# sara-nl/2D-VQ-AE-2

Hardware: AMD Instinct MI355X
Metric: patches/sec (VQAE.forward: encoder -> VQ -> decoder) (higher is better)
Workload: dtype f32; 1 GPU; BASELINE configs[1] (cfg B): batch 256/GPU of 256x256x3 fp32 -> 32x32 codes, K=256, D=128, full forward; global_batch=256, parallelism=patch-sharded x1

## Files before the change

### 2d-vq-ae-2_amd/csrc/conv_wino.hip

```cpp
#include "kernels.h"
#include "mfma.h"

namespace {

using namespace vqae;

struct WinoK {
    const float* __restrict__ t1;
    const float* __restrict__ U;
    const float* __restrict__ w3;
    const float* __restrict__ w1n;
    float* xio;
    float* y2;
    int H, Wimg, M;
    float act_a, act_b, t_scale, t_b4, n_b1a, n_b1b, n_b2a, n_b2b;
};

constexpr int BPF = 6;

template <int C> struct WinoCfg {
    static constexpr int W = C >= 128 ? 32 : (C == 64 ? 64 : 128);
    static constexpr int NT = C == 256 ? 512 : 256;
    static constexpr int NW = NT / 64;
    static constexpr int PX = 4 * W;
    static constexpr int TILES = PX / 4;
    static constexpr int TC = W / 2;
    static constexpr int NS = C / 32;
    static constexpr int KS = C / 8;
    static constexpr int C4 = C / 4;
    static constexpr int RP = NT / C4;
    static constexpr int LDT = C + 4;
    static constexpr int NI = C >= 64 ? 2 : 1;
    static constexpr int WN = C / (32 * NI);
    static constexpr int MI = PX / ((NW / WN) * 32);
    static constexpr int LDS_BYTES = PX * LDT * 4;
    static constexpr int PREF = C <= 64 ? 1 : 0;
};

template <int C, int TAIL, int DT, bool WIDE>
__global__ __launch_bounds__((WinoCfg<C>::NT), 2)
void wino_trunk_kernel(const WinoK p) {
    using K = WinoCfg<C>;
    auto rnd = [](float v) -> float {
        if (DT == VQAE_DT_BF16) return (float)(__bf16)v;
        if (DT == VQAE_DT_F16) return (float)(_Float16)v;
        return v;
    };
    auto rnd4 = [&](f32x4 v) -> f32x4 {
        if (DT != VQAE_DT_F32) {
#pragma unroll
            for (int e = 0; e < 4; ++e) v[e] = rnd(v[e]);
        }
        return v;
    };
    constexpr int W = K::W, PX = K::PX, TC = K::TC, NS = K::NS, KS = K::KS, C4 = K::C4, RP = K::RP, LDT = K::LDT, WN = K::WN;
    constexpr int MI = K::MI, NI = K::NI;
    constexpr bool PREF = K::PREF && !WIDE;
    constexpr int STEPS = 4 * KS;
    extern __shared__ __attribute__((aligned(16))) float lds[];
    const int tid = threadIdx.x;
    const int lane = tid & 63;
    const int wave = __builtin_amdgcn_readfirstlane(tid >> 6);
    const int li = lane & 31, hh = lane >> 5;
    const int ns = wave % NS, mt = wave / NS;

    int tile_m;
    {
        const int nwg = gridDim.x, bid = blockIdx.x;
        const int q = nwg >> 3, r = nwg & 7, xcd = bid & 7;
        tile_m = (xcd < r ? xcd * (q + 1) : r * (q + 1) + (xcd - r) * q) + (bid >> 3);
    }
    const int Wimg = WIDE ? p.Wimg : W;
    const int cblocks = WIDE ? p.Wimg / W : 1;
    const int tpi = (p.H / 4) * cblocks;
    const int img = tile_m / tpi;
    const int rem = tile_m - img * tpi;
    const int row0 = 4 * (rem / cblocks);
    const int col0 = W * (rem % cblocks);
    const int hw = p.H * Wimg;
    const float* const xim = p.t1 + (int64_t)img * hw * C;

    const int cg = tid % C4;
    const int tj0 = tid / C4;
    int coff[2][4], roff[2][4];
#pragma unroll
    for (int s = 0; s < 2; ++s) {
#pragma unroll
        for (int j = 0; j < 4; ++j) {
            int c = col0 + 2 * (tj0 + RP * s) - 1 + j;
            c = WIDE ? (c < 0 ? c + Wimg : (c >= Wimg ? c - Wimg : c)) : (c & (W - 1));
            coff[s][j] = c * C + 4 * cg;
            int r = row0 + 2 * s - 1 + j;
            r = r < 0 ? r + p.H : (r >= p.H ? r - p.H : r);
            roff[s][j] = r * Wimg * C;
        }
    }

    const float* const ub = p.U + (int64_t)ns * (KS * 256) + 4 * lane;
    const float* const af = lds + (mt * 32 + li) * LDT + 4 * hh;

    f32x4 v[4][4], la[2][4], lb[2][4];
    auto tr_load = [&](int xi, int s_r) {
        const int ra = xi == 0 ? 0 : (xi == 2 ? 2 : 1);
        const int rb = xi == 0 ? 2 : (xi == 1 ? 2 : (xi == 2 ? 1 : 3));
#pragma unroll
        for (int s_c = 0; s_c < 2; ++s_c)
#pragma unroll
            for (int j = 0; j < 4; ++j) {
                la[s_c][j] = rnd4(*reinterpret_cast<const f32x4*>(xim + roff[s_r][ra] + coff[s_c][j]));
                lb[s_c][j] = rnd4(*reinterpret_cast<const f32x4*>(xim + roff[s_r][rb] + coff[s_c][j]));
            }
    };
    auto tr_combine = [&](int xi, int s_r) {
#pragma unroll
        for (int s_c = 0; s_c < 2; ++s_c)
#pragma unroll
            for (int j = 0; j < 4; ++j)
                v[2 * s_r + s_c][j] = xi == 1 ? la[s_c][j] + lb[s_c][j] : la[s_c][j] - lb[s_c][j];
    };
    tr_load(0, 0);
    tr_combine(0, 0);
    tr_load(0, 1);
    tr_combine(0, 1);

    const int wm = wave / WN, wn = wave % WN;
    const int64_t pix0 = ((int64_t)img * p.H + row0) * Wimg + col0 + tj0;
    float* xr[4];
    f32x4 res[16];
    f32x4 bt[2][4][NI];
    auto tail_prefetch = [&](const float* __restrict__ wsrc) {
        const float* b0 = wsrc + (wn * NI) * (KS * 256) + 4 * lane;
#pragma unroll
        for (int u = 0; u < 4; ++u)
#pragma unroll
            for (int ni = 0; ni < NI; ++ni) bt[0][u][ni] = *reinterpret_cast<const f32x4*>(b0 + ni * (KS * 256) + 256 * u);
    };

    f32x16 y00, y01, y10, y11;
#pragma unroll
    for (int r = 0; r < 16; ++r) { y00[r] = 0.f; y01[r] = 0.f; y10[r] = 0.f; y11[r] = 0.f; }
#pragma unroll
    for (int xi = 0; xi < 4; ++xi) {
        __builtin_amdgcn_sched_barrier(0);
        if (xi > 0) __syncthreads();
#pragma unroll
        for (int it = 0; it < 4; ++it) {
            const int tile = (it >> 1) * TC + tj0 + RP * (it & 1);
            float* dst = lds + tile * LDT + 4 * cg;
            *reinterpret_cast<f32x4*>(dst + 0 * K::TILES * LDT) = v[it][0] - v[it][2];
            *reinterpret_cast<f32x4*>(dst + 1 * K::TILES * LDT) = v[it][1] + v[it][2];
            *reinterpret_cast<f32x4*>(dst + 2 * K::TILES * LDT) = v[it][2] - v[it][1];
            *reinterpret_cast<f32x4*>(dst + 3 * K::TILES * LDT) = v[it][1] - v[it][3];
        }

        const float* const ux = ub + (int64_t)(4 * xi) * (C * C);
#define WB(s) (((s) / KS) * (C * C) + 256 * ((s) % KS))
        f32x4 bq[BPF];
#pragma unroll
        for (int s = 0; s < BPF; ++s)
            bq[s] = *reinterpret_cast<const f32x4*>(ux + WB(s));
        __syncthreads();
        if (PREF && xi < 3) tr_load(xi + 1, 0);
        f32x4 aq[2];
        aq[0] = *reinterpret_cast<const f32x4*>(af);
#pragma unroll
        for (int nu = 0; nu < 4; ++nu) {
            f32x16 acc;
#pragma unroll
            for (int r = 0; r < 16; ++r) acc[r] = 0.f;
#pragma unroll
            for (int u = 0; u < KS; ++u) {
                const int s = KS * nu + u;
                if (s + 1 < STEPS)
                    aq[(s + 1) & 1] = *reinterpret_cast<const f32x4*>(af + ((s + 1) / KS) * K::TILES * LDT + 8 * ((s + 1) % KS));
                const f32x4 b = bq[s % BPF];
                if (s + BPF < STEPS)
                    bq[s % BPF] = *reinterpret_cast<const f32x4*>(ux + WB(s + BPF));
                if (xi == 3 && s == STEPS - BPF) {
                    tail_prefetch(p.w3);
#pragma unroll
                    for (int r = 0; r < 4; ++r) xr[r] = p.xio + (pix0 + (int64_t)r * Wimg) * C + 4 * cg;
#pragma unroll
                    for (int i = 0; i < 16; ++i) res[i] = __builtin_nontemporal_load(reinterpret_cast<const f32x4*>(xr[(RP * i) / W] + ((RP * i) % W) * C));
                }
#pragma unroll
                for (int r = 0; r < 4; ++r)
                    acc = __builtin_amdgcn_mfma_f32_32x32x2f32(b[r], aq[s & 1][r], acc, 0, 0, 0);
                __builtin_amdgcn_sched_barrier(0);
            }
            const int ca0 = xi <= 2 ? 1 : 0, ca1 = xi == 0 ? 0 : (xi == 1 ? 1 : -1);
            const int cb0 = nu <= 2 ? 1 : 0, cb1 = nu == 0 ? 0 : (nu == 1 ? 1 : -1);
            if (ca0 * cb0 != 0) y00 = y00 + acc;
            if (ca0 * cb1 == 1) y01 = y01 + acc; else if (ca0 * cb1 == -1) y01 = y01 - acc;
            if (ca1 * cb0 == 1) y10 = y10 + acc; else if (ca1 * cb0 == -1) y10 = y10 - acc;
            if (ca1 * cb1 == 1) y11 = y11 + acc; else if (ca1 * cb1 == -1) y11 = y11 - acc;
            asm volatile("" : "+v"(y00), "+v"(y01), "+v"(y10), "+v"(y11));
        }
#undef WB
        if (xi < 3) {
            if (!PREF) tr_load(xi + 1, 0);
            tr_combine(xi + 1, 0); tr_load(xi + 1, 1); tr_combine(xi + 1, 1);
        }
    }

    __syncthreads();
    float* const T = lds;
    {
        const int tile = mt * 32 + li;
        const int px = (2 * (tile / TC)) * W + 2 * (tile % TC);
        float* const d = T + px * LDT + 32 * ns + 4 * hh;
#pragma unroll
        for (int g = 0; g < 4; ++g) {
            f32x4 o00, o01, o10, o11;
#pragma unroll
            for (int e = 0; e < 4; ++e) {
                o00[e] = rnd(elu_act(rnd(y00[4 * g + e]) + p.act_a) + p.act_b);
                o01[e] = rnd(elu_act(rnd(y01[4 * g + e]) + p.act_a) + p.act_b);
                o10[e] = rnd(elu_act(rnd(y10[4 * g + e]) + p.act_a) + p.act_b);
                o11[e] = rnd(elu_act(rnd(y11[4 * g + e]) + p.act_a) + p.act_b);
            }
            *reinterpret_cast<f32x4*>(d + 8 * g) = o00;
            *reinterpret_cast<f32x4*>(d + 8 * g + LDT) = o01;
            *reinterpret_cast<f32x4*>(d + 8 * g + W * LDT) = o10;
            *reinterpret_cast<f32x4*>(d + 8 * g + (W + 1) * LDT) = o11;
        }
    }
    __syncthreads();

    f32x16 acc[MI][NI];
    auto gemm_tail = [&](const float* __restrict__ wsrc) {
#pragma unroll
        for (int mi = 0; mi < MI; ++mi)
#pragma unroll
            for (int ni = 0; ni < NI; ++ni)
#pragma unroll
                for (int r = 0; r < 16; ++r) acc[mi][ni][r] = 0.f;
        const float* a0 = T + (wm * MI * 32 + li) * LDT + 4 * hh;
        const float* b0 = wsrc + (wn * NI) * (KS * 256) + 4 * lane;
        f32x4 a[2][MI];
#pragma unroll
        for (int mi = 0; mi < MI; ++mi) a[0][mi] = *reinterpret_cast<const f32x4*>(a0 + mi * 32 * LDT);
#pragma unroll
        for (int ug = 0; ug < KS / 4; ++ug) {
            if (ug + 1 < KS / 4) {
#pragma unroll
                for (int u = 0; u < 4; ++u)
#pragma unroll
                    for (int ni = 0; ni < NI; ++ni)
                        bt[(ug + 1) & 1][u][ni] = *reinterpret_cast<const f32x4*>(b0 + ni * (KS * 256) + 256 * (4 * (ug + 1) + u));
            }
#pragma unroll
            for (int u = 0; u < 4; ++u) {
                const int ks = 4 * ug + u;
                if (ks + 1 < KS) {
#pragma unroll
                    for (int mi = 0; mi < MI; ++mi)
                        a[(ks + 1) & 1][mi] = *reinterpret_cast<const f32x4*>(a0 + mi * 32 * LDT + 8 * (ks + 1));
                }
#pragma unroll
                for (int r = 0; r < 4; ++r)
#pragma unroll
                    for (int mi = 0; mi < MI; ++mi)
#pragma unroll
                        for (int ni = 0; ni < NI; ++ni)
                            acc[mi][ni] = __builtin_amdgcn_mfma_f32_32x32x2f32(bt[ug & 1][u][ni][r], a[ks & 1][mi][r], acc[mi][ni], 0, 0, 0);
            }
        }
    };
    auto acc_to_lds = [&]() {
#pragma unroll
        for (int ni = 0; ni < NI; ++ni)
#pragma unroll
            for (int mi = 0; mi < MI; ++mi)
#pragma unroll
                for (int g = 0; g < 4; ++g) {
                    f32x4 o;
#pragma unroll
                    for (int e = 0; e < 4; ++e) o[e] = acc[mi][ni][4 * g + e];
                    *reinterpret_cast<f32x4*>(T + (wm * MI * 32 + mi * 32 + li) * LDT + (wn * NI + ni) * 32 + 8 * g + 4 * hh) = o;
                }
    };
    float* const trow = T + tj0 * LDT + 4 * cg;

    gemm_tail(p.w3);
    if (TAIL == 2) tail_prefetch(p.w1n);
    __syncthreads();
    acc_to_lds();
    __syncthreads();
#pragma unroll
    for (int i = 0; i < 16; ++i) {
        f32x4 t = rnd4(*reinterpret_cast<const f32x4*>(trow + RP * i * LDT));
        t = t * p.t_scale;
        t = t + p.t_b4;
        t = t + res[i];
        __builtin_nontemporal_store(t, reinterpret_cast<f32x4*>(xr[(RP * i) / W] + ((RP * i) % W) * C));
        if (TAIL == 2) {
#pragma unroll
            for (int e = 0; e < 4; ++e) t[e] = rnd(elu_act(t[e] + p.n_b1a) + p.n_b1b);
            *reinterpret_cast<f32x4*>(trow + RP * i * LDT) = t;
        }
    }
    if constexpr (TAIL == 2) {
        __syncthreads();
        gemm_tail(p.w1n);
        __syncthreads();
        acc_to_lds();
        __syncthreads();
        float* yr[4];
#pragma unroll
        for (int r = 0; r < 4; ++r) yr[r] = p.y2 + (pix0 + (int64_t)r * Wimg) * C + 4 * cg;
#pragma unroll
        for (int i = 0; i < 16; ++i) {
            f32x4 t = *reinterpret_cast<const f32x4*>(trow + RP * i * LDT);
#pragma unroll
            for (int e = 0; e < 4; ++e) t[e] = elu_act(rnd(t[e]) + p.n_b2a) + p.n_b2b;
            __builtin_nontemporal_store(t, reinterpret_cast<f32x4*>(yr[(RP * i) / W] + ((RP * i) % W) * C));
        }
    }
}

template <int C>
__global__ __launch_bounds__((WinoCfg<C>::NT), 2)
void fixup_conv1_kernel(const float* __restrict__ x, const float* __restrict__ w1f, float pa, float pb, float aa, float ab,
                        float* __restrict__ y) {
    using K = WinoCfg<C>;
    constexpr int PX = K::PX, KS = K::KS, C4 = K::C4, RP = K::RP, LDT = K::LDT, WN = K::WN, MI = K::MI, NI = K::NI;
    extern __shared__ __attribute__((aligned(16))) float lds[];
    float* const T = lds;
    const int tid = threadIdx.x;
    const int lane = tid & 63;
    const int wave = __builtin_amdgcn_readfirstlane(tid >> 6);
    const int li = lane & 31, hh = lane >> 5;
    const int cg = tid % C4, p0 = tid / C4;
    const int64_t m0 = (int64_t)blockIdx.x * PX;
    const float* const xrow = x + (m0 + p0) * C + 4 * cg;
    float* const trow = T + p0 * LDT + 4 * cg;
    f32x4 v[16];
#pragma unroll
    for (int i = 0; i < 16; ++i) v[i] = *reinterpret_cast<const f32x4*>(xrow + (int64_t)(RP * i) * C);
#pragma unroll
    for (int i = 0; i < 16; ++i) {
#pragma unroll
        for (int e = 0; e < 4; ++e) v[i][e] = elu_act(v[i][e] + pa) + pb;
        *reinterpret_cast<f32x4*>(trow + RP * i * LDT) = v[i];
    }
    __syncthreads();
    const int wm = wave / WN, wn = wave % WN;
    f32x16 acc[MI][NI];
#pragma unroll
    for (int mi = 0; mi < MI; ++mi)
#pragma unroll
        for (int ni = 0; ni < NI; ++ni)
#pragma unroll
            for (int r = 0; r < 16; ++r) acc[mi][ni][r] = 0.f;
    {
        const float* a0 = T + (wm * MI * 32 + li) * LDT + 4 * hh;
        const float* b0 = w1f + (wn * NI) * (KS * 256) + 4 * lane;
        f32x4 a[2][MI], bq[2][NI];
#pragma unroll
        for (int mi = 0; mi < MI; ++mi) a[0][mi] = *reinterpret_cast<const f32x4*>(a0 + mi * 32 * LDT);
#pragma unroll
        for (int ni = 0; ni < NI; ++ni) bq[0][ni] = *reinterpret_cast<const f32x4*>(b0 + ni * (KS * 256));
#pragma unroll
        for (int u = 0; u < KS; ++u) {
            if (u + 1 < KS) {
#pragma unroll
                for (int mi = 0; mi < MI; ++mi) a[(u + 1) & 1][mi] = *reinterpret_cast<const f32x4*>(a0 + mi * 32 * LDT + 8 * (u + 1));
#pragma unroll
                for (int ni = 0; ni < NI; ++ni) bq[(u + 1) & 1][ni] = *reinterpret_cast<const f32x4*>(b0 + ni * (KS * 256) + 256 * (u + 1));
            }
#pragma unroll
            for (int r = 0; r < 4; ++r)
#pragma unroll
                for (int mi = 0; mi < MI; ++mi)
#pragma unroll
                    for (int ni = 0; ni < NI; ++ni)
                        acc[mi][ni] = __builtin_amdgcn_mfma_f32_32x32x2f32(bq[u & 1][ni][r], a[u & 1][mi][r], acc[mi][ni], 0, 0, 0);
        }
    }
    __syncthreads();
#pragma unroll
    for (int ni = 0; ni < NI; ++ni)
#pragma unroll
        for (int mi = 0; mi < MI; ++mi)
#pragma unroll
            for (int g = 0; g < 4; ++g) {
                f32x4 o;
#pragma unroll
                for (int e = 0; e < 4; ++e) o[e] = elu_act(acc[mi][ni][4 * g + e] + aa) + ab;
                *reinterpret_cast<f32x4*>(T + (wm * MI * 32 + mi * 32 + li) * LDT + (wn * NI + ni) * 32 + 8 * g + 4 * hh) = o;
            }
    __syncthreads();
    float* const yrow = y + (m0 + p0) * C + 4 * cg;
#pragma unroll
    for (int i = 0; i < 16; ++i)
        *reinterpret_cast<f32x4*>(yrow + (int64_t)(RP * i) * C) = *reinterpret_cast<const f32x4*>(trow + RP * i * LDT);
}

template <int C>
__global__ __launch_bounds__((WinoCfg<C>::NT), 2)
void fixup_conv1p_kernel(const float* __restrict__ x, const float* __restrict__ w1f, float pa, float pb, float aa, float ab,
                         float* __restrict__ y, const int n_tiles) {
    using K = WinoCfg<C>;
    constexpr int PX = K::PX, KS = K::KS, C4 = K::C4, RP = K::RP, LDT = K::LDT, WN = K::WN, MI = K::MI, NI = K::NI;
    extern __shared__ __attribute__((aligned(16))) float lds[];
    float* const T = lds;
    const int tid = threadIdx.x;
    const int lane = tid & 63;
    const int wave = __builtin_amdgcn_readfirstlane(tid >> 6);
    const int li = lane & 31, hh = lane >> 5;
    const int cg = tid % C4, p0 = tid / C4;
    const int wm = wave / WN, wn = wave % WN;
    float* const trow = T + p0 * LDT + 4 * cg;
    const float* const a0 = T + (wm * MI * 32 + li) * LDT + 4 * hh;
    const float* const b0 = w1f + (wn * NI) * (KS * 256) + 4 * lane;
    int tile = blockIdx.x;
    f32x4 v[16];
    if (tile < n_tiles) {
        const float* const xrow = x + ((int64_t)tile * PX + p0) * C + 4 * cg;
#pragma unroll
        for (int i = 0; i < 16; ++i) v[i] = __builtin_nontemporal_load(reinterpret_cast<const f32x4*>(xrow + (int64_t)(RP * i) * C));
    }
    for (; tile < n_tiles; tile += gridDim.x) {
#pragma unroll
        for (int i = 0; i < 16; ++i) {
#pragma unroll
            for (int e = 0; e < 4; ++e) v[i][e] = elu_act(v[i][e] + pa) + pb;
            *reinterpret_cast<f32x4*>(trow + RP * i * LDT) = v[i];
        }
        vqae::lds_barrier();
        const int nt = tile + gridDim.x;
        if (nt < n_tiles) {
            const float* const xrow = x + ((int64_t)nt * PX + p0) * C + 4 * cg;
#pragma unroll
            for (int i = 0; i < 16; ++i) v[i] = __builtin_nontemporal_load(reinterpret_cast<const f32x4*>(xrow + (int64_t)(RP * i) * C));
        }
        f32x16 acc[MI][NI];
#pragma unroll
        for (int mi = 0; mi < MI; ++mi)
#pragma unroll
            for (int ni = 0; ni < NI; ++ni)
#pragma unroll
                for (int r = 0; r < 16; ++r) acc[mi][ni][r] = 0.f;
        {
            f32x4 a[2][MI], bq[2][NI];
#pragma unroll
            for (int mi = 0; mi < MI; ++mi) a[0][mi] = *reinterpret_cast<const f32x4*>(a0 + mi * 32 * LDT);
#pragma unroll
            for (int ni = 0; ni < NI; ++ni) bq[0][ni] = *reinterpret_cast<const f32x4*>(b0 + ni * (KS * 256));
#pragma unroll 1
            for (int u2 = 0; u2 < KS; u2 += 2) {
#pragma unroll
                for (int uu = 0; uu < 2; ++uu) {
                    const int u = u2 + uu;
                    if (u + 1 < KS) {
#pragma unroll
                        for (int mi = 0; mi < MI; ++mi) a[(uu + 1) & 1][mi] = *reinterpret_cast<const f32x4*>(a0 + mi * 32 * LDT + 8 * (u + 1));
#pragma unroll
                        for (int ni = 0; ni < NI; ++ni) bq[(uu + 1) & 1][ni] = *reinterpret_cast<const f32x4*>(b0 + ni * (KS * 256) + 256 * (u + 1));
                    }
#pragma unroll
                    for (int r = 0; r < 4; ++r)
#pragma unroll
                        for (int mi = 0; mi < MI; ++mi)
#pragma unroll
                            for (int ni = 0; ni < NI; ++ni)
                                acc[mi][ni] = __builtin_amdgcn_mfma_f32_32x32x2f32(bq[uu & 1][ni][r], a[uu & 1][mi][r], acc[mi][ni], 0, 0, 0);
                }
            }
        }
        vqae::lds_barrier();
#pragma unroll
        for (int ni = 0; ni < NI; ++ni)
#pragma unroll
            for (int mi = 0; mi < MI; ++mi)
#pragma unroll
                for (int g = 0; g < 4; ++g) {
                    f32x4 o;
#pragma unroll
                    for (int e = 0; e < 4; ++e) o[e] = elu_act(acc[mi][ni][4 * g + e] + aa) + ab;
                    *reinterpret_cast<f32x4*>(T + (wm * MI * 32 + mi * 32 + li) * LDT + (wn * NI + ni) * 32 + 8 * g + 4 * hh) = o;
                }
        vqae::lds_barrier();
        float* const yrow = y + ((int64_t)tile * PX + p0) * C + 4 * cg;
#pragma unroll
        for (int i = 0; i < 16; ++i)
            *reinterpret_cast<f32x4*>(yrow + (int64_t)(RP * i) * C) = *reinterpret_cast<const f32x4*>(trow + RP * i * LDT);
        vqae::lds_barrier();
    }
}

__global__ void wino_weight_kernel(const float* __restrict__ w, int c, int dt, float* __restrict__ U) {
    const int i = blockIdx.x * blockDim.x + threadIdx.x;
    if (i >= c * c) return;
    float g[3][3], t[4][3];
#pragma unroll
    for (int a = 0; a < 3; ++a)
#pragma unroll
        for (int b = 0; b < 3; ++b) g[a][b] = vqae::round_dt(w[(int64_t)i * 9 + a * 3 + b], dt);
#pragma unroll
    for (int b = 0; b < 3; ++b) {
        t[0][b] = g[0][b];
        t[1][b] = 0.5f * (g[0][b] + g[1][b] + g[2][b]);
        t[2][b] = 0.5f * (g[0][b] - g[1][b] + g[2][b]);
        t[3][b] = g[2][b];
    }
    const int fo = frag_offset(i / c, i % c, c);
    const int64_t cc = (int64_t)c * c;
#pragma unroll
    for (int a = 0; a < 4; ++a) {
        U[(a * 4 + 0) * cc + fo] = t[a][0];
        U[(a * 4 + 1) * cc + fo] = 0.5f * (t[a][0] + t[a][1] + t[a][2]);
        U[(a * 4 + 2) * cc + fo] = 0.5f * (t[a][0] - t[a][1] + t[a][2]);
        U[(a * 4 + 3) * cc + fo] = t[a][2];
    }
}

__global__ void frag_weight_kernel(const float* __restrict__ w, int n_rows, int K, int sk, float* __restrict__ out) {
    const int i = blockIdx.x * blockDim.x + threadIdx.x;
    if (i >= n_rows * K) return;
    out[frag_offset(i / K, i % K, K, sk)] = w[i];
}

template <int C, int DT, bool WIDE>
int launch_wino_w(const WinoK& k, bool chain, hipStream_t stream) {
    using K = WinoCfg<C>;
    if (int rc = vqae::set_max_dynamic_lds((const void*)wino_trunk_kernel<C, 1, DT, WIDE>, K::LDS_BYTES)) return rc;
    if (int rc = vqae::set_max_dynamic_lds((const void*)wino_trunk_kernel<C, 2, DT, WIDE>, K::LDS_BYTES)) return rc;
    const unsigned grid = (unsigned)(k.M / K::PX);
    const double flops = 2.0 * (double)k.M * C * (4.0 * C + C + (chain ? C : 0));
    vqae::ProfScope prof(C >= 128 ? vqae::PROF_CONV3X3_TRUNK : vqae::PROF_NONE, stream, flops);
    if (chain) wino_trunk_kernel<C, 2, DT, WIDE><<<grid, K::NT, K::LDS_BYTES, stream>>>(k);
    else wino_trunk_kernel<C, 1, DT, WIDE><<<grid, K::NT, K::LDS_BYTES, stream>>>(k);
    prof.done();
    VQAE_LAUNCH_CHECK();
    return VQAE_OK;
}

template <int C, int DT = VQAE_DT_F32>
int launch_wino(const WinoK& k, bool chain, hipStream_t stream) {
    return k.Wimg == WinoCfg<C>::W ? launch_wino_w<C, DT, false>(k, chain, stream) : launch_wino_w<C, DT, true>(k, chain, stream);
}

}

namespace vqae {

bool wino_trunk_channels(int c, int dtype) { return dtype == VQAE_DT_F32 ? (c == 256 || c == 128 || c == 64 || c == 32) : c == 32; }

bool wino_trunk_supported(int c, int h, int w, int dtype) {
    if (!wino_trunk_channels(c, dtype)) return false;
    const int span = c >= 128 ? 32 : (c == 64 ? WinoCfg<64>::W : WinoCfg<32>::W);
    return w >= span && w % span == 0 && h >= 4 && h % 4 == 0;
}

size_t wino_weight_floats(int c) { return (size_t)16 * c * c; }

int wino_transform_weight(const float* w_oihw_dev, int c, int dtype, float* U_dev, hipStream_t stream) {
    wino_weight_kernel<<<(unsigned)ceil_div(c * c, 256), 256, 0, stream>>>(w_oihw_dev, c, dtype, U_dev);
    VQAE_LAUNCH_CHECK();
    return VQAE_OK;
}

bool fixup_conv1_supported(int c, int64_t m) {
    if (c != 256 && c != 128 && c != 64 && c != 32) return false;
    const int px = c >= 128 ? 128 : (c == 64 ? WinoCfg<64>::PX : WinoCfg<32>::PX);
    return m > 0 && m % px == 0;
}

template <int C>
static int launch_conv1(const float* x, const float* w1f, float pa, float pb, float aa, float ab, float* y, int64_t m,
                        hipStream_t stream) {
    using K = WinoCfg<C>;
    if (int rc = set_max_dynamic_lds((const void*)fixup_conv1_kernel<C>, K::LDS_BYTES)) return rc;
    if (int rc = set_max_dynamic_lds((const void*)fixup_conv1p_kernel<C>, K::LDS_BYTES)) return rc;
    const int n_cu = cu_count();
    const bool oneshot = env_int("VQAE_CONV1_ONESHOT", 0) != 0;
    const int64_t n_tiles = m / K::PX;
    const int wgs = (int)std::min<int64_t>((K::LDS_BYTES * 2 <= 160 * 1024 ? 2 : 1) * n_cu, n_tiles);
    const int64_t min_tiles = env_int("VQAE_CONV1_PERSIST_MIN_TILES", 4ll * n_cu);
    ProfScope prof(C >= 128 ? PROF_CONV1X1_TRUNK : PROF_NONE, stream, 2.0 * (double)m * C * C);
    if (oneshot || C > 128 || n_tiles < min_tiles)
        fixup_conv1_kernel<C><<<(unsigned)n_tiles, K::NT, K::LDS_BYTES, stream>>>(x, w1f, pa, pb, aa, ab, y);
    else
        fixup_conv1p_kernel<C><<<(unsigned)wgs, K::NT, K::LDS_BYTES, stream>>>(x, w1f, pa, pb, aa, ab, y, (int)n_tiles);
    prof.done();
    VQAE_LAUNCH_CHECK();
    return VQAE_OK;
}

int fixup_conv1(const float* x, const float* w1f, float pa, float pb, float aa, float ab, float* y, int64_t m, int c,
                hipStream_t stream) {
    VQAE_REQUIRE(x && w1f && y, VQAE_ERR_INVALID, "fixup_conv1: null pointer");
    VQAE_REQUIRE(fixup_conv1_supported(c, m), VQAE_ERR_UNSUPPORTED, "fixup_conv1: C = %d, M = %lld", c, (long long)m);
    VQAE_REQUIRE(m / 128 < (1ll << 31), VQAE_ERR_UNSUPPORTED, "fixup_conv1: too many pixels");
    if (c == 256) return launch_conv1<256>(x, w1f, pa, pb, aa, ab, y, m, stream);
    if (c == 128) return launch_conv1<128>(x, w1f, pa, pb, aa, ab, y, m, stream);
    if (c == 64) return launch_conv1<64>(x, w1f, pa, pb, aa, ab, y, m, stream);
    return launch_conv1<32>(x, w1f, pa, pb, aa, ab, y, m, stream);
}

int frag_weight(const float* w_packed_dev, int n_rows, int K, int sk, float* out_dev, hipStream_t stream) {
    VQAE_REQUIRE(n_rows % 32 == 0 && (sk == 8 || sk == 16) && K % sk == 0, VQAE_ERR_INVALID, "frag_weight: %d x %d, k-slice %d", n_rows, K, sk);
    frag_weight_kernel<<<(unsigned)ceil_div((int64_t)n_rows * K, 256), 256, 0, stream>>>(w_packed_dev, n_rows, K, sk, out_dev);
    VQAE_LAUNCH_CHECK();
    return VQAE_OK;
}

int wino_trunk_tail(const float* t1, const float* U, const float* w3, float act_a, float act_b, float t_scale, float t_b4,
                    float* xio, const NextConv1& next, int batch, int h, int w, int c, int dtype, hipStream_t stream) {
    if (batch == 0) return VQAE_OK;
    const float* w1n = (const float*)next.w1;
    float* t1_next = (float*)next.t1_next;
    VQAE_REQUIRE(t1 && U && w3 && xio && (!w1n || t1_next), VQAE_ERR_INVALID, "wino_trunk_tail: null pointer");
    VQAE_REQUIRE(wino_trunk_supported(c, h, w, dtype), VQAE_ERR_UNSUPPORTED, "wino_trunk_tail: C = %d, H = %d, W = %d, dtype %d", c, h, w, dtype);
    const int64_t M = (int64_t)batch * h * w;
    VQAE_REQUIRE(M < (1ll << 31) - 256, VQAE_ERR_UNSUPPORTED, "wino_trunk_tail: too many pixels");
    WinoK k;
    memset(&k, 0, sizeof(k));
    k.t1 = t1; k.U = U; k.w3 = w3; k.w1n = w1n; k.xio = xio; k.y2 = t1_next;
    k.H = h; k.Wimg = w; k.M = (int)M;
    k.act_a = act_a; k.act_b = act_b; k.t_scale = t_scale; k.t_b4 = t_b4;
    k.n_b1a = next.b1a; k.n_b1b = next.b1b; k.n_b2a = next.b2a; k.n_b2b = next.b2b;
    return dtype == VQAE_DT_BF16 ? launch_wino<32, VQAE_DT_BF16>(k, w1n != nullptr, stream)
         : dtype == VQAE_DT_F16 ? launch_wino<32, VQAE_DT_F16>(k, w1n != nullptr, stream)
         : c == 256 ? launch_wino<256>(k, w1n != nullptr, stream)
         : c == 128 ? launch_wino<128>(k, w1n != nullptr, stream)
         : (c == 64 ? launch_wino<64>(k, w1n != nullptr, stream) : launch_wino<32>(k, w1n != nullptr, stream));
}

}
```

Measured before the change: 4556 patches/s.

## Stage raw input rows in an LDS ring for C=32 Winograd trunk

For the C=32 non-wide Winograd trunk kernel, raw input rows are staged into a 4-slot LDS ring buffer instead of computing the input transform in registers and writing transformed tiles to LDS. The Winograd input transform is then applied on the fly from ring reads inside the MFMA loop, with only the needed columns loaded per step. Row loads are issued early and ring writes happen only at xi=1 and xi=3, with lighter LDS barriers replacing full syncthreads. The aim is less global re-reading of overlapping rows, fewer LDS writes and cheaper synchronisation, at the cost of extra VALU combine work and register pressure in the inner loop.

```diff
diff --git a/2d-vq-ae-2_amd/csrc/conv_wino.hip b/2d-vq-ae-2_amd/csrc/conv_wino.hip
--- a/2d-vq-ae-2_amd/csrc/conv_wino.hip
+++ b/2d-vq-ae-2_amd/csrc/conv_wino.hip
@@ -35,6 +35,9 @@
     static constexpr int MI = PX / ((NW / WN) * 32);
     static constexpr int LDS_BYTES = PX * LDT * 4;
     static constexpr int PREF = C <= 64 ? 1 : 0;
+    static constexpr int ROW_LDS = W * LDT;
+    static constexpr int ring_px(int px) { return px * LDT + ((px & 16) ? 4 : 0); }
+    static constexpr int ring_slot(int rel) { return rel == 0 ? 0 : (rel == -1 || rel == 2 ? 1 : (rel == 3 ? 3 : 2)); }
 };
 
 template <int C, int TAIL, int DT, bool WIDE>
@@ -55,8 +58,10 @@
     };
     constexpr int W = K::W, PX = K::PX, TC = K::TC, NS = K::NS, KS = K::KS, C4 = K::C4, RP = K::RP, LDT = K::LDT, WN = K::WN;
     constexpr int MI = K::MI, NI = K::NI;
-    constexpr bool PREF = K::PREF && !WIDE;
+    constexpr bool ROWS = C == 32 && !WIDE;
+    constexpr bool PREF = K::PREF && !WIDE && !ROWS;
     constexpr int STEPS = 4 * KS;
+    static_assert(!ROWS || (4 * K::ROW_LDS * 4 == K::LDS_BYTES && K::NS == 1 && K::TC == 64 && K::RP * 4 == W), "ring geometry");
     extern __shared__ __attribute__((aligned(16))) float lds[];
     const int tid = threadIdx.x;
     const int lane = tid & 63;
@@ -118,10 +123,65 @@
             for (int j = 0; j < 4; ++j)
                 v[2 * s_r + s_c][j] = xi == 1 ? la[s_c][j] + lb[s_c][j] : la[s_c][j] - lb[s_c][j];
     };
-    tr_load(0, 0);
-    tr_combine(0, 0);
-    tr_load(0, 1);
-    tr_combine(0, 1);
+    if constexpr (!ROWS) {
+        tr_load(0, 0);
+        tr_combine(0, 0);
+        tr_load(0, 1);
+        tr_combine(0, 1);
+    }
+
+    f32x4 stg[4], raw[2][4], rc[ROWS ? KS : 1][4];
+    const float* fr[4];
+    float* ring_w;
+    if constexpr (ROWS) {
+        ring_w = lds + K::ring_px(tj0) + 4 * cg;
+#pragma unroll
+        for (int j = 0; j < 4; ++j)
+            fr[j] = lds + (mt >> 1) * K::ROW_LDS + K::ring_px((2 * ((mt & 1) * 32 + li) - 1 + j) & (W - 1)) + 4 * hh;
+    }
+    auto stage_load = [&](int rel, f32x4* dst) {
+        int r = row0 + rel;
+        r = r < 0 ? r + p.H : (r >= p.H ? r - p.H : r);
+        const float* const src = xim + r * (W * C) + tj0 * C + 4 * cg;
+#pragma unroll
+        for (int i = 0; i < 4; ++i) dst[i] = *reinterpret_cast<const f32x4*>(src + RP * i * C);
+    };
+    auto stage_write = [&](int rel, const f32x4* src) {
+#pragma unroll
+        for (int i = 0; i < 4; ++i)
+            *reinterpret_cast<f32x4*>(ring_w + K::ring_slot(rel) * K::ROW_LDS + RP * i * LDT) = rnd4(src[i]);
+    };
+    auto rows_need = [](int xi, int nu) -> int {
+        return xi < 3 ? (nu == 0 ? 15 : 0) : (nu == 0 ? 5 : (nu == 1 ? 6 : (nu == 2 ? 0 : 10)));
+    };
+    auto rows_read = [&](int xi, int u, int cols) {
+        const int ra = xi == 0 ? 0 : (xi == 2 ? 2 : 1);
+        const int rb = xi == 0 ? 2 : (xi == 1 ? 2 : (xi == 2 ? 1 : 3));
+        const int oa = K::ring_slot(ra - 1) * K::ROW_LDS + 8 * u, ob = K::ring_slot(rb - 1) * K::ROW_LDS + 8 * u;
+#pragma unroll
+        for (int j = 0; j < 4; ++j)
+            if (cols >> j & 1) {
+                raw[0][j] = *reinterpret_cast<const f32x4*>(fr[j] + oa);
+                raw[1][j] = *reinterpret_cast<const f32x4*>(fr[j] + ob);
+            }
+    };
+    auto rows_combine = [&](int xi, int u, int cols) {
+#pragma unroll
+        for (int j = 0; j < 4; ++j)
+            if (cols >> j & 1) rc[u][j] = xi == 1 ? raw[0][j] + raw[1][j] : raw[0][j] - raw[1][j];
+    };
+    auto rows_operand = [&](int nu, int u) -> f32x4 {
+        return nu == 0 ? rc[u][0] - rc[u][2] : (nu == 1 ? rc[u][1] + rc[u][2] : (nu == 2 ? rc[u][2] - rc[u][1] : rc[u][1] - rc[u][3]));
+    };
+    if constexpr (ROWS) {
+        f32x4 st[4][4];
+        constexpr int first[4] = {-1, 1, 3, 0};
+#pragma unroll
+        for (int q = 0; q < 4; ++q) stage_load(first[q], st[q]);
+        stage_load(2, stg);
+#pragma unroll
+        for (int q = 0; q < 4; ++q) stage_write(first[q], st[q]);
+    }
 
     const int wm = wave / WN, wn = wave % WN;
     const int64_t pix0 = ((int64_t)img * p.H + row0) * Wimg + col0 + tj0;
@@ -142,15 +202,22 @@
 #pragma unroll
     for (int xi = 0; xi < 4; ++xi) {
         __builtin_amdgcn_sched_barrier(0);
-        if (xi > 0) __syncthreads();
-#pragma unroll
-        for (int it = 0; it < 4; ++it) {
-            const int tile = (it >> 1) * TC + tj0 + RP * (it & 1);
-            float* dst = lds + tile * LDT + 4 * cg;
-            *reinterpret_cast<f32x4*>(dst + 0 * K::TILES * LDT) = v[it][0] - v[it][2];
-            *reinterpret_cast<f32x4*>(dst + 1 * K::TILES * LDT) = v[it][1] + v[it][2];
-            *reinterpret_cast<f32x4*>(dst + 2 * K::TILES * LDT) = v[it][2] - v[it][1];
-            *reinterpret_cast<f32x4*>(dst + 3 * K::TILES * LDT) = v[it][1] - v[it][3];
+        if constexpr (ROWS) {
+            if (xi == 1 || xi == 3) {
+                vqae::lds_barrier();
+                stage_write(xi + 1, stg);
+            }
+        } else {
+            if (xi > 0) __syncthreads();
+#pragma unroll
+            for (int it = 0; it < 4; ++it) {
+                const int tile = (it >> 1) * TC + tj0 + RP * (it & 1);
+                float* dst = lds + tile * LDT + 4 * cg;
+                *reinterpret_cast<f32x4*>(dst + 0 * K::TILES * LDT) = v[it][0] - v[it][2];
+                *reinterpret_cast<f32x4*>(dst + 1 * K::TILES * LDT) = v[it][1] + v[it][2];
+                *reinterpret_cast<f32x4*>(dst + 2 * K::TILES * LDT) = v[it][2] - v[it][1];
+                *reinterpret_cast<f32x4*>(dst + 3 * K::TILES * LDT) = v[it][1] - v[it][3];
+            }
         }
 
         const float* const ux = ub + (int64_t)(4 * xi) * (C * C);
@@ -159,10 +226,17 @@
 #pragma unroll
         for (int s = 0; s < BPF; ++s)
             bq[s] = *reinterpret_cast<const f32x4*>(ux + WB(s));
-        __syncthreads();
-        if (PREF && xi < 3) tr_load(xi + 1, 0);
         f32x4 aq[2];
-        aq[0] = *reinterpret_cast<const f32x4*>(af);
+        if constexpr (ROWS) {
+            if (xi != 2) vqae::lds_barrier();
+            else stage_load(4, stg);
+            rows_read(xi, 0, rows_need(xi, 0));
+            rows_combine(xi, 0, rows_need(xi, 0));
+        } else {
+            __syncthreads();
+            if (PREF && xi < 3) tr_load(xi + 1, 0);
+            aq[0] = *reinterpret_cast<const f32x4*>(af);
+        }
 #pragma unroll
         for (int nu = 0; nu < 4; ++nu) {
             f32x16 acc;
@@ -171,8 +245,12 @@
 #pragma unroll
             for (int u = 0; u < KS; ++u) {
                 const int s = KS * nu + u;
-                if (s + 1 < STEPS)
+                if constexpr (ROWS) {
+                    if (s + 1 < STEPS) rows_read(xi, (s + 1) % KS, rows_need(xi, (s + 1) / KS));
+                    aq[s & 1] = rows_operand(nu, u);
+                } else if (s + 1 < STEPS) {
                     aq[(s + 1) & 1] = *reinterpret_cast<const f32x4*>(af + ((s + 1) / KS) * K::TILES * LDT + 8 * ((s + 1) % KS));
+                }
                 const f32x4 b = bq[s % BPF];
                 if (s + BPF < STEPS)
                     bq[s % BPF] = *reinterpret_cast<const f32x4*>(ux + WB(s + BPF));
@@ -186,6 +264,12 @@
 #pragma unroll
                 for (int r = 0; r < 4; ++r)
                     acc = __builtin_amdgcn_mfma_f32_32x32x2f32(b[r], aq[s & 1][r], acc, 0, 0, 0);
+                if constexpr (ROWS) {
+                    if (s + 1 < STEPS && rows_need(xi, (s + 1) / KS) != 0) {
+                        __builtin_amdgcn_sched_barrier(0);
+                        rows_combine(xi, (s + 1) % KS, rows_need(xi, (s + 1) / KS));
+                    }
+                }
                 __builtin_amdgcn_sched_barrier(0);
             }
             const int ca0 = xi <= 2 ? 1 : 0, ca1 = xi == 0 ? 0 : (xi == 1 ? 1 : -1);
@@ -197,7 +281,7 @@
             asm volatile("" : "+v"(y00), "+v"(y01), "+v"(y10), "+v"(y11));
         }
 #undef WB
-        if (xi < 3) {
+        if (!ROWS && xi < 3) {
             if (!PREF) tr_load(xi + 1, 0);
             tr_combine(xi + 1, 0); tr_load(xi + 1, 1); tr_combine(xi + 1, 1);
         }
```

Result: faster. 4602 patches/s (median of 6 runs) (+1.0%).
